# 959AI994/Multi-Gate-VAE

Hardware: NVIDIA B200
Metric: gates_per_s_fwd_bwd (higher is better)
Workload: dtype f32

## Files before the change

### multi-gate-vae_b200/csrc/mgv_tc.cuh

```cuda
#pragma once
#include <cuda_fp16.h>
#include "mgv_common.cuh"

namespace tc {

__device__ __forceinline__ uint32_t smem_u32(const void* p) { return (uint32_t)__cvta_generic_to_shared(p); }

__device__ __forceinline__ uint32_t sw128_off(int r, int c16) {
    return (uint32_t)((r >> 3) * 1024 + (r & 7) * 128 + ((c16 ^ (r & 7)) << 4));
}
__device__ __forceinline__ uint32_t plain16_off(int r, int c16) {
    return (uint32_t)((r >> 3) * 256 + c16 * 128 + (r & 7) * 16);
}

__device__ __forceinline__ uint32_t pack_f16x2_sat(float e0, float e1) {
    uint32_t r;
    asm("cvt.rn.satfinite.f16x2.f32 %0, %1, %2;" : "=r"(r) : "f"(e1), "f"(e0));
    return r;
}
__device__ __forceinline__ void split2(float a, float b, uint32_t& hi, uint32_t& lo) {
    hi = pack_f16x2_sat(a, b);
    const float2 hf = __half22float2(*reinterpret_cast<const __half2*>(&hi));
    lo = pack_f16x2_sat(a - hf.x, b - hf.y);
}
// ... 41 lines not shown
        if ((++polls & 1023u) == 0u) {
            const unsigned long long now = global_timer_ns();
            if (t0 == 0ull) t0 = now;
            else if (now - t0 > WAIT_TIMEOUT_NS) __trap();
        }
    }
};
__device__ __forceinline__ bool mbar_try_wait(uint32_t bar, uint32_t parity) {
    uint32_t done;
    asm volatile(
        "{\n\t.reg .pred p;\n\t"
        "mbarrier.try_wait.parity.shared::cta.b64 p, [%1], %2;\n\t"
        "selp.b32 %0, 1, 0, p;\n\t}"
        : "=r"(done) : "r"(bar), "r"(parity) : "memory");
    return done != 0u;
}
__device__ __forceinline__ void mbar_wait(uint32_t bar, uint32_t parity) {
    WaitGuard g;
#pragma unroll 1
    while (!mbar_try_wait(bar, parity)) g.tick();
}

__device__ __forceinline__ void mbar_wait_warp(uint32_t bar, uint32_t parity, int lane, unsigned sleep_ns = 64) {
    if (lane == 0) {
        WaitGuard g;
#pragma unroll 1
        while (!mbar_try_wait(bar, parity)) {
            if (sleep_ns) __nanosleep(sleep_ns);
            g.tick();
        }
    }
    __syncwarp();
}
__device__ __forceinline__ void mbar_wait_sleep(uint32_t bar, uint32_t parity, unsigned sleep_ns = 64) {
    WaitGuard g;
#pragma unroll 1
    while (!mbar_try_wait(bar, parity)) {
        __nanosleep(sleep_ns);
        g.tick();
    }
}

__device__ __forceinline__ void mbar_expect_tx(uint32_t bar, uint32_t bytes) {
    asm volatile("{\n\t.reg .b64 st;\n\tmbarrier.arrive.expect_tx.shared::cta.b64 st, [%0], %1;\n\t}" ::"r"(bar), "r"(bytes) : "memory");
}
__device__ __forceinline__ void bulk_g2s(uint32_t dst, const void* src, uint32_t bytes, uint32_t bar) {
    asm volatile("cp.async.bulk.shared::cluster.global.mbarrier::complete_tx::bytes [%0], [%1], %2, [%3];"
                 ::"r"(dst), "l"(src), "r"(bytes), "r"(bar) : "memory");
}

__device__ __forceinline__ void bulk_s2g(void* dst, uint32_t src, uint32_t bytes) {
    asm volatile("cp.async.bulk.global.shared::cta.bulk_group [%0], [%1], %2;" ::"l"(dst), "r"(src), "r"(bytes) : "memory");
}
__device__ __forceinline__ uint64_t l2_policy_evict_first() {
    uint64_t pol;
    asm volatile("createpolicy.fractional.L2::evict_first.b64 %0, 1.0;" : "=l"(pol));
    return pol;
}
__device__ __forceinline__ void bulk_s2g_hint(void* dst, uint32_t src, uint32_t bytes, uint64_t pol) {
    asm volatile("cp.async.bulk.global.shared::cta.bulk_group.L2::cache_hint [%0], [%1], %2, %3;" ::"l"(dst), "r"(src), "r"(bytes), "l"(pol) : "memory");
}
__device__ __forceinline__ void bulk_g2s_hint(uint32_t dst, const void* src, uint32_t bytes, uint32_t bar, uint64_t pol) {
    asm volatile("cp.async.bulk.shared::cluster.global.mbarrier::complete_tx::bytes.L2::cache_hint [%0], [%1], %2, [%3], %4;"
                 ::"r"(dst), "l"(src), "r"(bytes), "r"(bar), "l"(pol) : "memory");
}
__device__ __forceinline__ void stg_v4_hint(void* dst, const uint4& v, uint64_t pol) {
    asm volatile("st.global.L2::cache_hint.v4.b32 [%0], {%1,%2,%3,%4}, %5;" ::"l"(dst), "r"(v.x), "r"(v.y), "r"(v.z), "r"(v.w), "l"(pol) : "memory");
}
__device__ __forceinline__ void bulk_commit() { asm volatile("cp.async.bulk.commit_group;" ::: "memory"); }
__device__ __forceinline__ void bulk_wait_read0() { asm volatile("cp.async.bulk.wait_group.read 0;" ::: "memory"); }
__device__ __forceinline__ void bulk_wait0() { asm volatile("cp.async.bulk.wait_group 0;" ::: "memory"); }
__device__ __forceinline__ void named_bar_sync(int id, int nthreads) {
    asm volatile("bar.sync %0, %1;" ::"r"(id), "r"(nthreads) : "memory");
}
__device__ __forceinline__ void tmem_ld8(uint32_t taddr, float (&v)[8]) {
    uint32_t* r = reinterpret_cast<uint32_t*>(v);
    asm volatile("tcgen05.ld.sync.aligned.32x32b.x8.b32 {%0,%1,%2,%3,%4,%5,%6,%7}, [%8];"
                 : "=r"(r[0]), "=r"(r[1]), "=r"(r[2]), "=r"(r[3]), "=r"(r[4]), "=r"(r[5]), "=r"(r[6]), "=r"(r[7])
                 : "r"(taddr) : "memory");
}

__device__ __forceinline__ void fence_async_smem() { asm volatile("fence.proxy.async.shared::cta;" ::: "memory"); }
__device__ __forceinline__ void fence_before_sync() { asm volatile("tcgen05.fence::before_thread_sync;" ::: "memory"); }
__device__ __forceinline__ void fence_after_sync() { asm volatile("tcgen05.fence::after_thread_sync;" ::: "memory"); }

__device__ __forceinline__ void tmem_alloc(uint32_t* slot, uint32_t ncols) {
    asm volatile("tcgen05.alloc.cta_group::1.sync.aligned.shared::cta.b32 [%0], %1;" ::"r"(smem_u32(slot)), "r"(ncols) : "memory");
    asm volatile("tcgen05.relinquish_alloc_permit.cta_group::1.sync.aligned;" ::: "memory");
}
__device__ __forceinline__ void tmem_dealloc(uint32_t base, uint32_t ncols) {
    asm volatile("tcgen05.dealloc.cta_group::1.sync.aligned.b32 %0, %1;" ::"r"(base), "r"(ncols) : "memory");
}
__device__ __forceinline__ void tmem_ld32(uint32_t taddr, float (&v)[32]) {
    uint32_t* r = reinterpret_cast<uint32_t*>(v);
    asm volatile(
        "tcgen05.ld.sync.aligned.32x32b.x32.b32 "
        "{%0,%1,%2,%3,%4,%5,%6,%7,%8,%9,%10,%11,%12,%13,%14,%15,"
        "%16,%17,%18,%19,%20,%21,%22,%23,%24,%25,%26,%27,%28,%29,%30,%31}, [%32];"
        : "=r"(r[0]), "=r"(r[1]), "=r"(r[2]), "=r"(r[3]), "=r"(r[4]), "=r"(r[5]), "=r"(r[6]), "=r"(r[7]),
          "=r"(r[8]), "=r"(r[9]), "=r"(r[10]), "=r"(r[11]), "=r"(r[12]), "=r"(r[13]), "=r"(r[14]), "=r"(r[15]),
          "=r"(r[16]), "=r"(r[17]), "=r"(r[18]), "=r"(r[19]), "=r"(r[20]), "=r"(r[21]), "=r"(r[22]), "=r"(r[23]),
          "=r"(r[24]), "=r"(r[25]), "=r"(r[26]), "=r"(r[27]), "=r"(r[28]), "=r"(r[29]), "=r"(r[30]), "=r"(r[31])
        : "r"(taddr) : "memory");
}
__device__ __forceinline__ void tmem_ld16(uint32_t taddr, float (&v)[16]) {
    uint32_t* r = reinterpret_cast<uint32_t*>(v);
// ... 136 lines not shown
```

### multi-gate-vae_b200/csrc/struct_bwd_tc.cu

```cuda
#include <stdlib.h>
#include "struct_layout.cuh"

long long* mgv_debug_trace();
size_t mgv_struct_image_bytes(int num_enc);
int mgv_struct_build_image(const float* weights, int num_enc, uint8_t* image, int precision, cudaStream_t st);

namespace {
using namespace struct_layout;

constexpr int SGRAD = MGV_STRUCT_GRAD_FLOATS;
constexpr int EPI_WARPS = 8, GATHER_WARPS = 8;
constexpr int THREADS = (EPI_WARPS + GATHER_WARPS + 1) * 32;
constexpr int LDGS = 68;
constexpr uint32_t DG_TILE_BYTES = 131072;
constexpr int CHUNK_TILES_DEFAULT = 2048;

constexpr uint32_t S_G = A_X_LO + 4096;
constexpr uint32_t S_LN = S_G + TM * LDGS * 4;
constexpr uint32_t S_AMAX = S_LN + 512;
constexpr uint32_t S_EX = S_AMAX + 16;
constexpr uint32_t S_BAR = S_EX + 4 * 2 * TM * 4;
constexpr uint32_t S_TMEM = S_BAR + 128;
constexpr uint32_t P_SMEM = S_TMEM + 64 + 1024;
static_assert(P_SMEM <= 227 * 1024, "struct backward: shared memory");
static_assert(A_TILE_BYTES + TM * LDGS * 4 >= TM * 132 * 4, "LayerNorm gradient scratch aliases the tile + staging");
constexpr uint32_t T_ACC = 0, T_OUT = 256, T_LNP = 384;

struct BwdTC {
    int N, feat, layernorm, first, last, dir;
    int tile_beg, tile_end;
    const int* ptr;
    const int* idx;
    const int* order;
    const int* gdesc;
    const unsigned* tile_cost;
    const float* x;
    const uint8_t* image;
    const float* gout;
    const float* in_part; const float* in_agg;
    float* out_part; float* out_agg;
    const uint8_t* tiles;
    size_t tiles_enc_stride;
    uint8_t* dgbuf;
    float* scales;
    unsigned* smin;
    float* partial;
    int gxp;
    int chunk_cap;
    long long* trace;
};
#define PTRACE_MAX(slot) do { if (p.trace && it < 16) atomicMax(reinterpret_cast<unsigned long long*>(p.trace) + (((size_t)blockIdx.y * gridDim.x + blockIdx.x) * 16 + it) * 16 + (slot), (unsigned long long)clock64()); } while (0)
#define PTRACE(slot) do { if (p.trace && it < 16) p.trace[(((size_t)blockIdx.y * gridDim.x + blockIdx.x) * 16 + it) * 16 + (slot)] = clock64(); } while (0)

__device__ __forceinline__ float4 lds4(const float* p) { return *reinterpret_cast<const float4*>(p); }
__device__ __forceinline__ float pow2_scale(float amax) {
    if (!(amax > 0.f) || !isfinite(amax)) return 1.0f;
    const int e = (int)((__float_as_uint(amax) >> 23) & 0xff) - 127;
    int k = 8 - e;
    k = k < -100 ? -100 : (k > 100 ? 100 : k);
    return __uint_as_float((uint32_t)(k + 127) << 23);
}
__device__ __forceinline__ float pow2_scale_keep(float amax, float cur) {
    const float v = amax * cur;
    if (v >= 4.0f && v <= 8192.0f) return cur;
    return (amax > 0.f) ? pow2_scale(amax) : cur;
}

template <bool LOWP>
__global__ void __launch_bounds__(THREADS, 1) struct_bwd_pw_kernel(const BwdTC p) {
    extern __shared__ __align__(1024) uint8_t smem_raw[];
    const uint32_t sbase = (tc::smem_u32(smem_raw) + 1023u) & ~1023u;
    uint8_t* sgen = smem_raw + (sbase - tc::smem_u32(smem_raw));
    const int tid = threadIdx.x, lane = tid & 31, warp = tid >> 5;
    const int enc = blockIdx.y;
    const size_t eoff = (size_t)enc * p.N * D;
    const uint8_t* image = p.image + (size_t)enc * 2 * IMG_BYTES;

    const uint32_t bar_w = sbase + S_BAR, bar_a_full = bar_w + 8, bar_t_full = bar_w + 16, bar_g_empty = bar_w + 24;
    const uint32_t bar_acc_full = bar_w + 32, bar_out_full = bar_w + 40, bar_h_read = bar_w + 48, bar_dg_full = bar_w + 56;
    const uint32_t bar_dg_stored = bar_w + 64;
    uint32_t* tmem_slot = reinterpret_cast<uint32_t*>(sgen + S_TMEM);
    float* s_ln = reinterpret_cast<float*>(sgen + S_LN);
    unsigned* s_amax = reinterpret_cast<unsigned*>(sgen + S_AMAX);
    float* s_g = reinterpret_cast<float*>(sgen + S_G);

    if (tid == 0) {
        tc::mbar_init(bar_w, 1);
        tc::mbar_init(bar_a_full, GATHER_WARPS * 32);
        tc::mbar_init(bar_t_full, 1);
        tc::mbar_init(bar_g_empty, EPI_WARPS * 32);
        tc::mbar_init(bar_acc_full, 1);
        tc::mbar_init(bar_out_full, 1);
        tc::mbar_init(bar_h_read, EPI_WARPS * 32);
        tc::mbar_init(bar_dg_full, EPI_WARPS * 32);
        tc::mbar_init(bar_dg_stored, EPI_WARPS * 32);
        tc::fence_barrier_init();
        tc::mbar_expect_tx(bar_w, IMG_W);
#pragma unroll 1
        for (uint32_t o = 0; o < IMG_W; o += 16384u) tc::bulk_g2s(sbase + o, image + o, 16384u, bar_w);
    }
    if (tid < 2 * D) s_ln[tid] = __ldg(reinterpret_cast<const float*>(image + IMG_W) + tid);
    if (tid < 4) s_amax[tid] = 0u;
    if (warp == 0) tc::tmem_alloc(tmem_slot, 512);
    const int tile_beg = p.tile_beg + (int)blockIdx.x, tile_end = p.tile_end, tile_step = (int)gridDim.x;
    tc::fence_before_sync();
    __syncthreads();
    tc::fence_after_sync();
    const uint32_t tmem = *tmem_slot;

    if (warp >= EPI_WARPS && warp < EPI_WARPS + GATHER_WARPS) {
        const int gw = warp - EPI_WARPS, rg = lane >> 3, c = lane & 7;
        const int4* gdesc = reinterpret_cast<const int4*>(p.gdesc);
        const float* gsrc = p.last ? p.gout + eoff : p.in_part + eoff;
        const float* asrc = p.in_agg + eoff;
        const bool nbg = !p.last;
        int4 dn[4];
#pragma unroll
        for (int ps = 0; ps < 4; ++ps) {
            const int r = tile_beg * TM + gw * 16 + ps * 4 + rg;
            dn[ps] = (tile_beg < tile_end && r < p.N) ? __ldg(gdesc + r) : make_int4(-1, 0, 0, 0);
        }
        int it = 0;
        for (int tile = tile_beg; tile < tile_end; tile += tile_step, ++it) {
            if (lane == 0) PTRACE_MAX(13);
            int4 dc[4];
#pragma unroll
            for (int ps = 0; ps < 4; ++ps) dc[ps] = dn[ps];
#pragma unroll
            for (int ps = 0; ps < 4; ++ps) {
                const int r = (tile + tile_step) * TM + gw * 16 + ps * 4 + rg;
                dn[ps] = (tile + tile_step < tile_end && r < p.N) ? __ldg(gdesc + r) : make_int4(-1, 0, 0, 0);
            }
#pragma unroll
            for (int hf = 0; hf < 2; ++hf) {
                int node[2], beg[2], cnt[2], jn[2];
                float4 g[2][2], va[2][2];
                int maxc = 0;
                const float4 z4 = make_float4(0.f, 0.f, 0.f, 0.f);
#pragma unroll
                for (int q = 0; q < 2; ++q) {
                    const int4 d = dc[2 * hf + q];
                    node[q] = d.x; beg[q] = d.y; cnt[q] = nbg ? d.z : 0; jn[q] = d.w;
                    maxc = max(maxc, cnt[q]);
                    g[q][0] = z4; g[q][1] = z4; va[q][0] = z4; va[q][1] = z4;
                    if (node[q] >= 0) {
                        g[q][0] = mgv_ld4(gsrc + (size_t)node[q] * D + c * 8);
                        g[q][1] = mgv_ld4(gsrc + (size_t)node[q] * D + c * 8 + 4);
                    }
                    if (cnt[q] > 0) {
                        va[q][0] = mgv_ld4(asrc + (size_t)jn[q] * D + c * 8);
                        va[q][1] = mgv_ld4(asrc + (size_t)jn[q] * D + c * 8 + 4);
                    }
                    if (cnt[q] > 1) jn[q] = p.idx[beg[q] + 1] & NODE_MASK;
                }
                float ag[2][8];
#pragma unroll
                for (int q = 0; q < 2; ++q) {
                    ag[q][0] = g[q][0].x + va[q][0].x; ag[q][1] = g[q][0].y + va[q][0].y; ag[q][2] = g[q][0].z + va[q][0].z; ag[q][3] = g[q][0].w + va[q][0].w;
                    ag[q][4] = g[q][1].x + va[q][1].x; ag[q][5] = g[q][1].y + va[q][1].y; ag[q][6] = g[q][1].z + va[q][1].z; ag[q][7] = g[q][1].w + va[q][1].w;
                }
                for (int sl = 1; sl < maxc; sl += 2) {
                    int j[2][2];
#pragma unroll
                    for (int q = 0; q < 2; ++q) {
                        j[q][0] = jn[q];
                        j[q][1] = (sl + 1 < cnt[q]) ? (p.idx[beg[q] + sl + 1] & NODE_MASK) : 0;
                        if (sl + 2 < cnt[q]) jn[q] = p.idx[beg[q] + sl + 2] & NODE_MASK;
                    }
                    float4 wa[2][2][2];
#pragma unroll
                    for (int q = 0; q < 2; ++q)
#pragma unroll
                        for (int t = 0; t < 2; ++t) {
                            wa[q][t][0] = z4; wa[q][t][1] = z4;
                            if (sl + t < cnt[q]) {
                                wa[q][t][0] = mgv_ld4(asrc + (size_t)j[q][t] * D + c * 8);
                                wa[q][t][1] = mgv_ld4(asrc + (size_t)j[q][t] * D + c * 8 + 4);
                            }
                        }
#pragma unroll
                    for (int q = 0; q < 2; ++q)
#pragma unroll
                        for (int t = 0; t < 2; ++t) {
                            ag[q][0] += wa[q][t][0].x; ag[q][1] += wa[q][t][0].y; ag[q][2] += wa[q][t][0].z; ag[q][3] += wa[q][t][0].w;
                            ag[q][4] += wa[q][t][1].x; ag[q][5] += wa[q][t][1].y; ag[q][6] += wa[q][t][1].z; ag[q][7] += wa[q][t][1].w;
                        }
                }
                if (hf == 0) {
                    if (lane == 0) PTRACE_MAX(14);
                    tc::mbar_wait_warp(bar_g_empty, (uint32_t)((it & 1) ^ 1), lane, 64);
                }
#pragma unroll
                for (int q = 0; q < 2; ++q) {
                    float* dst = s_g + (gw * 16 + (2 * hf + q) * 4 + rg) * LDGS + c * 8;
                    *reinterpret_cast<float4*>(dst) = make_float4(ag[q][0], ag[q][1], ag[q][2], ag[q][3]);
                    *reinterpret_cast<float4*>(dst + 4) = make_float4(ag[q][4], ag[q][5], ag[q][6], ag[q][7]);
                }
            }
            tc::mbar_arrive(bar_a_full);
            if (lane == 0) PTRACE_MAX(15);
        }
    } else if (warp == EPI_WARPS + GATHER_WARPS) {
        if (lane == 0 && tile_beg < tile_end) {
            auto load_tile = [&](int t) {
                const uint8_t* src = p.tiles + (size_t)enc * p.tiles_enc_stride + (size_t)t * A_TILE_BYTES;
                if (LOWP) {
                    tc::mbar_expect_tx(bar_t_full, 36864u);
#pragma unroll 1
                    for (uint32_t o = 0; o < 16384u; o += 8192u) {
                        tc::bulk_g2s(sbase + A_AGG_HI + o, src + o, 8192u, bar_t_full);
                        tc::bulk_g2s(sbase + A_H_HI + o, src + (A_H_HI - A_AGG_HI) + o, 8192u, bar_t_full);
                    }
                    tc::bulk_g2s(sbase + A_X_HI, src + (A_X_HI - A_AGG_HI), 4096u, bar_t_full);
                } else {
                    tc::mbar_expect_tx(bar_t_full, A_TILE_BYTES);
#pragma unroll 1
                    for (uint32_t o = 0; o < A_TILE_BYTES; o += 8192u) tc::bulk_g2s(sbase + A_AGG_HI + o, src + o, 8192u, bar_t_full);
                }
            };
            auto issue_recompute = [&](uint32_t tph) {
                tc::mbar_wait_sleep(bar_t_full, tph, 32);
                tc::fence_after_sync();
                const uint32_t d = tmem + T_ACC;
                tc::mma3p<LOWP>(d, tc::desc_k_plain16(sbase + A_X_HI), tc::desc_k_plain16(sbase + A_X_LO),
                         tc::desc_k_plain16(sbase + WX_HI), tc::desc_k_plain16(sbase + WX_LO), tc::make_idesc(128, 256, false, false, LOWP), 0u);
#pragma unroll
                for (int j = 0; j < 4; ++j)
                    tc::mma3p<LOWP>(d, tc::desc_k_sw128(sbase + A_H_HI + 32 * j), tc::desc_k_sw128(sbase + A_H_LO + 32 * j),
                             tc::desc_k_sw128(sbase + WHH_HI + 32 * j), tc::desc_k_sw128(sbase + WHH_LO + 32 * j),
                             tc::make_idesc(128, 128, false, false, LOWP), 1u);
#pragma unroll
                for (int j = 0; j < 4; ++j)
                    tc::mma3p<LOWP>(d + 192u, tc::desc_k_sw128(sbase + A_H_HI + 32 * j), tc::desc_k_sw128(sbase + A_H_LO + 32 * j),
                             tc::desc_k_sw128(sbase + WHH_HI + 16384 + 32 * j), tc::desc_k_sw128(sbase + WHH_LO + 16384 + 32 * j),
                             tc::make_idesc(128, 64, false, false, LOWP), 1u);
#pragma unroll
                for (int j = 0; j < 4; ++j)
                    tc::mma3p<LOWP>(d, tc::desc_k_sw128(sbase + A_AGG_HI + 32 * j), tc::desc_k_sw128(sbase + A_AGG_LO + 32 * j),
                             tc::desc_k_sw128(sbase + WC_HI + 32 * j), tc::desc_k_sw128(sbase + WC_LO + 32 * j),
                             tc::make_idesc(128, 192, false, false, LOWP), 1u);
                tc::mma_commit(bar_acc_full);
            };
            tc::mbar_wait_sleep(bar_w, 0u);
            load_tile(tile_beg);
            issue_recompute(0u);
            int it = 0;
            for (int tile = tile_beg; tile < tile_end; tile += tile_step, ++it) {
                const uint32_t ph = (uint32_t)(it & 1);
                tc::mbar_wait_sleep(bar_acc_full, ph, 32);
                tc::mbar_wait_sleep(bar_h_read, ph, 32);
                if (tile + tile_step < tile_end) load_tile(tile + tile_step);
                tc::mbar_wait_sleep(bar_dg_full, ph, 32);
                tc::fence_after_sync();
                PTRACE(7);
                if (!p.first) {
                    const uint32_t o = tmem + T_OUT;
                    const uint32_t i128 = tc::make_idesc(128, 128, false, true, LOWP), i64 = tc::make_idesc(128, 64, false, true, LOWP);
#pragma unroll
                    for (int s = 0; s < 8; ++s) {
                        const uint32_t a = tmem + T_ACC + 16u * s;
                        tc::mma3p_ts<LOWP>(o, a, a + 8u, tc::desc_mn_sw128(sbase + WC_HI + 2048u * s, WHH_HI - WC_HI),
                                            tc::desc_mn_sw128(sbase + WC_LO + 2048u * s, WHH_LO - WC_LO), i128, 1u);
                    }
#pragma unroll
                    for (int s = 8; s < 12; ++s) {
                        const uint32_t a = tmem + T_ACC + 16u * s;
                        tc::mma3p_ts<LOWP>(o, a, a + 8u, tc::desc_mn_sw128(sbase + WC_HI + 2048u * s, 0),
                                            tc::desc_mn_sw128(sbase + WC_LO + 2048u * s, 0), i64, 1u);
                    }
#pragma unroll
                    for (int s = 12; s < 16; ++s) {
                        const uint32_t a = tmem + T_ACC + 16u * s;
                        tc::mma3p_ts<LOWP>(o + 64u, a, a + 8u, tc::desc_mn_sw128(sbase + WHH_HI + 2048u * (s - 4), 0),
                                            tc::desc_mn_sw128(sbase + WHH_LO + 2048u * (s - 4), 0), i64, 1u);
                    }
                    tc::mma_commit(bar_out_full);
                }
                if (tile + tile_step < tile_end) {
                    tc::mbar_wait_sleep(bar_dg_stored, ph, 32);
                    issue_recompute(ph ^ 1u);
                }
                PTRACE(3);
            }
        }
    } else if (warp < EPI_WARPS) {
        const int wg = warp >> 2, row = (warp & 3) * 32 + lane, u0 = 32 * wg;
        const uint32_t tl = tmem + ((uint32_t)((warp & 3) * 32) << 16);
        const uint32_t t_acc = tl + T_ACC, t_out = tl + T_OUT, t_lnp = tl + T_LNP;
        const float* gs = s_g + row * LDGS;
        float* s_ex = reinterpret_cast<float*>(sgen + S_EX);
        constexpr int EPI_T = EPI_WARPS * 32;
#pragma unroll 1
        for (int cc = 0; cc < 32; cc += 4) {
            tc::tmem_st4(t_lnp + u0 + cc, 0.f, 0.f, 0.f, 0.f);
            tc::tmem_st4(t_lnp + 64 + u0 + cc, 0.f, 0.f, 0.f, 0.f);
        }
        tc::tmem_st_wait();
        float run_scale = 1.0f;
        const uint64_t pol_stream = tc::l2_policy_evict_first();
        int it = 0;
        for (int tile = tile_beg; tile < tile_end; tile += tile_step, ++it) {
            const uint32_t ph = (uint32_t)(it & 1);
            const bool valid = tile * TM + row < p.N;
            const int node = valid ? p.order[tile * TM + row] : 0;
            tc::mbar_wait_warp(bar_t_full, ph, lane, 32);
#pragma unroll
            for (int c8 = 0; c8 < 4; ++c8) {
                const uint32_t off = tc::sw128_off(row, 4 * wg + c8);
                const uint4 hi = *reinterpret_cast<const uint4*>(sgen + A_H_HI + off);
                float h[8];
                if (LOWP) {
                    const uint32_t* w = reinterpret_cast<const uint32_t*>(&hi);
#pragma unroll
                    for (int e = 0; e < 4; ++e) { h[2 * e] = __uint_as_float(w[e] << 16); h[2 * e + 1] = __uint_as_float(w[e] & 0xffff0000u); }
                } else {
                    const uint4 lo = *reinterpret_cast<const uint4*>(sgen + A_H_LO + off);
                    const __half2* h2 = reinterpret_cast<const __half2*>(&hi);
                    const __half2* l2 = reinterpret_cast<const __half2*>(&lo);
#pragma unroll
                    for (int e = 0; e < 4; ++e) {
                        const float2 a = __half22float2(h2[e]), bq = __half22float2(l2[e]);
                        h[2 * e] = a.x + bq.x; h[2 * e + 1] = a.y + bq.y;
                    }
                }
                tc::tmem_st8f(t_out + u0 + 8 * c8, h);
            }
            tc::mbar_arrive(bar_h_read);
            tc::mbar_wait_warp(bar_acc_full, ph, lane, 32);
            tc::mbar_wait_warp(bar_a_full, ph, lane, 32);
            tc::fence_after_sync();
            tc::tmem_st_wait();
            if (tid == 0) PTRACE(4);
            float sum = 0.f;
#pragma unroll 1
            for (int c8 = 0; c8 < 4; ++c8) {
                const int u = u0 + 8 * c8;
                float gr[8], gz[8], gi[8], gh[8], h[8];
                tc::tmem_ld8(t_acc + u, gr);
                tc::tmem_ld8(t_acc + 64 + u, gz);
                tc::tmem_ld8(t_acc + 128 + u, gi);
                tc::tmem_ld8(t_acc + 192 + u, gh);
                tc::tmem_ld8(t_out + u, h);
                tc::tmem_ld_wait();
#pragma unroll
                for (int e = 0; e < 8; ++e) {
                    float r, z, n, hn;
                    gru_gates(gr[e], gz[e], gi[e], gh[e], r, z, n, hn);
                    gr[e] = r; gz[e] = z; gi[e] = n;
                    h[e] = fmaf(z, h[e] - n, n);
                    sum += h[e];
                }
                tc::tmem_st8f(t_acc + u, gr);
                tc::tmem_st8f(t_acc + 64 + u, gz);
                tc::tmem_st8f(t_acc + 128 + u, gi);
// ... 151 lines not shown
                    tc::stg_v4_hint(hb + 3072, make_uint4(qk[4], qk[5], qk[6], qk[7]), pol_stream);
                    if (!LOWP) {
                        tc::stg_v4_hint(hb + 65536, make_uint4(pk[8], pk[9], pk[10], pk[11]), pol_stream);
                        tc::stg_v4_hint(hb + 65536 + 1024, make_uint4(pk[12], pk[13], pk[14], pk[15]), pol_stream);
                        tc::stg_v4_hint(hb + 65536 + 2048, make_uint4(qk[8], qk[9], qk[10], qk[11]), pol_stream);
                        tc::stg_v4_hint(hb + 65536 + 3072, make_uint4(qk[12], qk[13], qk[14], qk[15]), pol_stream);
                    }
                }
            }
            tc::fence_before_sync();
            tc::mbar_arrive(bar_dg_stored);
            if (!p.first) {
                tc::mbar_wait_warp(bar_out_full, ph, lane, 32);
                tc::fence_after_sync();
                if (tid == 0) PTRACE(8);
                const float inv = 1.0f / scale;
#pragma unroll 2
                for (int c8 = 0; c8 < 4; ++c8) {
                    const int u = u0 + 8 * c8;
                    float a[8], q[8];
                    tc::tmem_ld8(t_out + u, a);
                    tc::tmem_ld8(t_out + 64 + u, q);
                    tc::tmem_ld_wait();
#pragma unroll
                    for (int e = 0; e < 8; ++e) { a[e] *= inv; q[e] *= inv; }
                    if (valid) {
                        stg8(p.out_agg + eoff + (size_t)node * D + u, a);
                        stg8(p.out_part + eoff + (size_t)node * D + u, q);
                    }
                }
            }
            if (tid == 0) PTRACE(9);
        }
    }
    tc::fence_before_sync();
    __syncthreads();
    tc::fence_after_sync();
    float* scratch = reinterpret_cast<float*>(sgen + A_AGG_HI);
    if (warp < EPI_WARPS) {
        const int row = (warp & 3) * 32 + lane, u0 = 32 * (warp >> 2);
        const uint32_t t_lnp = tmem + ((uint32_t)((warp & 3) * 32) << 16) + T_LNP;
#pragma unroll 1
        for (int c8 = 0; c8 < 8; ++c8) {
            const int col = (c8 < 4) ? u0 + 8 * c8 : 64 + u0 + 8 * (c8 - 4);
            float v[8];
            tc::tmem_ld8(t_lnp + col, v);
            tc::tmem_ld_wait();
            *reinterpret_cast<float4*>(scratch + row * 132 + col) = make_float4(v[0], v[1], v[2], v[3]);
            *reinterpret_cast<float4*>(scratch + row * 132 + col + 4) = make_float4(v[4], v[5], v[6], v[7]);
        }
    }
    tc::fence_before_sync();
    __syncthreads();
    if (tid < 2 * D && p.layernorm && tile_beg < tile_end) {
        float s = 0.f;
#pragma unroll 8
        for (int r = 0; r < TM; ++r) s += scratch[r * 132 + tid];
        float* part = p.partial + (((size_t)enc * p.gxp + blockIdx.x) * 2 + p.dir) * SGRAD;
        part[O_LNW + tid] += s;
    }
    if (warp == 0) tc::tmem_dealloc(tmem, 512);
}

__device__ __forceinline__ void red_add4(float4* dst, const float4& v) {
    asm volatile("red.global.add.v4.f32 [%0], {%1,%2,%3,%4};" ::"l"(dst), "f"(v.x), "f"(v.y), "f"(v.z), "f"(v.w) : "memory");
}

constexpr int W_THREADS = 6 * 32;
constexpr uint32_t ST_DG_HI = 0, ST_DG_LO = 32768, ST_AGG_HI = 65536, ST_H_HI = 73728, ST_AGG_LO = 81920, ST_H_LO = 90112;
constexpr uint32_t ST_X_HI = 98304, ST_X_LO = 100352, ST_BYTES = 102400;
constexpr uint32_t W_BAR = 2 * ST_BYTES;
constexpr uint32_t W_TMEM = W_BAR + 64;
constexpr uint32_t W_SMEM = W_TMEM + 64 + 1024;
static_assert(W_SMEM <= 227 * 1024, "struct weight gradient: shared memory");

struct WgTC {
    int ntiles;
    int chunk_cap;
    int dir, gxp;
    const uint8_t* tiles;
    size_t tiles_enc_stride;
    int tile_base;
    const uint8_t* dgbuf;
    const float* scales;
    const unsigned* smin;
    float* partial;
    long long* trace;
};
#define WTRACE(slot) do { if (p.trace && i < 16) p.trace[(((size_t)blockIdx.y * gridDim.x + blockIdx.x) * 16 + i) * 16 + (slot)] = clock64(); } while (0)

template <bool LOWP>
__global__ void __launch_bounds__(W_THREADS, 1) struct_bwd_wgrad_kernel(const WgTC p) {
    extern __shared__ __align__(1024) uint8_t smem_raw[];
    const uint32_t sbase = (tc::smem_u32(smem_raw) + 1023u) & ~1023u;
    uint8_t* sgen = smem_raw + (sbase - tc::smem_u32(smem_raw));
    const int tid = threadIdx.x, lane = tid & 31, warp = tid >> 5;
    const int enc = blockIdx.y;
    const uint32_t bar_full = sbase + W_BAR, bar_ready = bar_full + 16, bar_empty = bar_full + 32, bar_done = bar_full + 48;
    uint32_t* tmem_slot = reinterpret_cast<uint32_t*>(sgen + W_TMEM);
    if (tid == 0) {
        for (int s = 0; s < 2; ++s) {
            tc::mbar_init(bar_full + 8 * s, 1);
            tc::mbar_init(bar_ready + 8 * s, 4 * 32);
            tc::mbar_init(bar_empty + 8 * s, 1);
        }
        tc::mbar_init(bar_done, 1);
        tc::fence_barrier_init();
    }
    if (warp == 0) tc::tmem_alloc(tmem_slot, 512);
    tc::fence_before_sync();
    __syncthreads();
    tc::fence_after_sync();
    const uint32_t tmem = *tmem_slot;
    const int tile_beg = (int)((long long)p.ntiles * blockIdx.x / gridDim.x);
    const int tile_end = (int)((long long)p.ntiles * (blockIdx.x + 1) / gridDim.x);
    const int nhalf = 2 * (tile_end - tile_beg);
    const float smin = __uint_as_float(p.smin[enc]);

    if (warp == 0) {
        if (lane == 0) {
            const uint64_t pol = tc::l2_policy_evict_first();
            for (int i = 0; i < nhalf; ++i) {
                const int s = i & 1, tile = tile_beg + (i >> 1), h = i & 1;
                WTRACE(0);
                tc::mbar_wait_sleep(bar_empty + 8 * s, (uint32_t)(((i >> 1) & 1) ^ 1));
                WTRACE(1);
                tc::mbar_expect_tx(bar_full + 8 * s, LOWP ? 51200u : ST_BYTES);
                const uint8_t* dg = p.dgbuf + ((size_t)enc * p.chunk_cap + tile) * DG_TILE_BYTES + (size_t)h * 32768;
                const uint8_t* at = p.tiles + (size_t)enc * p.tiles_enc_stride + (size_t)(p.tile_base + tile) * A_TILE_BYTES;
                const uint32_t st = sbase + (uint32_t)s * ST_BYTES, bar = bar_full + 8 * s;
                tc::bulk_g2s_hint(st + ST_DG_HI, dg, 16384u, bar, pol);
                tc::bulk_g2s_hint(st + ST_DG_HI + 16384u, dg + 16384, 16384u, bar, pol);
                tc::bulk_g2s_hint(st + ST_AGG_HI, at + 0 + h * 8192, 8192u, bar, pol);
                tc::bulk_g2s_hint(st + ST_H_HI, at + 32768 + h * 8192, 8192u, bar, pol);
                tc::bulk_g2s_hint(st + ST_X_HI, at + 65536 + h * 2048, 2048u, bar, pol);
                if (!LOWP) {
                    tc::bulk_g2s_hint(st + ST_DG_LO, dg + 65536, 16384u, bar, pol);
                    tc::bulk_g2s_hint(st + ST_DG_LO + 16384u, dg + 65536 + 16384, 16384u, bar, pol);
                    tc::bulk_g2s_hint(st + ST_AGG_LO, at + 16384 + h * 8192, 8192u, bar, pol);
                    tc::bulk_g2s_hint(st + ST_H_LO, at + 49152 + h * 8192, 8192u, bar, pol);
                    tc::bulk_g2s_hint(st + ST_X_LO, at + 69632 + h * 2048, 2048u, bar, pol);
                }
            }
        }
    } else if (warp == 1) {
        if (lane == 0) {
            const uint32_t i128 = tc::make_idesc(128, 128, true, true, LOWP), i16 = tc::make_idesc(128, 16, true, true, LOWP);
            for (int i = 0; i < nhalf; ++i) {
                const int s = i & 1;
                WTRACE(4);
                tc::mbar_wait_sleep(bar_ready + 8 * s, (uint32_t)((i >> 1) & 1), 32);
                tc::fence_after_sync();
                WTRACE(5);
                const uint32_t st = sbase + (uint32_t)s * ST_BYTES;
#pragma unroll
                for (int j = 0; j < 4; ++j) {
                    const uint32_t acc = (i > 0 || j > 0) ? 1u : 0u;
                    const uint64_t b_hi = tc::desc_mn_sw128(st + ST_AGG_HI + 2048u * j, 8192), b_lo = tc::desc_mn_sw128(st + ST_AGG_LO + 2048u * j, 8192);
                    const uint64_t x_hi = tc::desc_mn_plain16(st + ST_X_HI + 512u * j), x_lo = tc::desc_mn_plain16(st + ST_X_LO + 512u * j);
#pragma unroll
                    for (int g = 0; g < 2; ++g) {
                        const uint64_t a_hi = tc::make_desc(st + ST_DG_HI + 16384u * g + 256u * j, 128, 1024, tc::LAYOUT_NONE);
                        const uint64_t a_lo = tc::make_desc(st + ST_DG_LO + 16384u * g + 256u * j, 128, 1024, tc::LAYOUT_NONE);
                        tc::mma3p<LOWP>(tmem + 160u * g, a_hi, a_lo, b_hi, b_lo, i128, acc);
                        tc::mma3p<LOWP>(tmem + 160u * g + 128u, a_hi, a_lo, x_hi, x_lo, i16, acc);
                    }
// ... 53 lines not shown
            for (int q = t128; q < G3 * 19; q += 128) {
                const int o = q / 19, c4 = q % 19;
                if (c4 < 18) {
                    const int g = o >= 128 ? 1 : 0, col = c4 < 16 ? 4 * c4 : 128 + 4 * (c4 - 16);
                    const float4 v = *reinterpret_cast<const float4*>(stg + (g * 128 + o - 128 * g) * FLD + col);
                    red_add4(part4 + (O_WCX + o * LDC) / 4 + c4, v);
                }
            }
            for (int q = t128; q < G3 * 17; q += 128) {
                const int o = q / 17, c4 = q % 17;
                if (c4 < 16) {
                    const int row = o >= 128 ? 128 + o - 64 : o;
                    const float4 v = *reinterpret_cast<const float4*>(stg + row * FLD + 64 + 4 * c4);
                    red_add4(part4 + (O_WHH + o * LDM) / 4 + c4, v);
                }
            }
            for (int o = t128; o < G3; o += 128) {
                const int rc = o >= 128 ? 128 + o - 128 : o, rh = o >= 128 ? 128 + o - 64 : o;
                atomicAdd(part + O_BC + o, stg[rc * FLD + 136]);
                atomicAdd(part + O_BIH + o, stg[rc * FLD + 137]);
                atomicAdd(part + O_BHH + o, stg[rh * FLD + 137]);
            }
            if (tid == 64) WTRACE(10);
        }
    }
    tc::fence_before_sync();
    __syncthreads();
    if (warp == 0) tc::tmem_dealloc(tmem, 512);
}

__global__ void struct_reduce_tc_kernel(const float* __restrict__ partial, int gxp, float* __restrict__ grads, int num_enc) {
    const size_t total = (size_t)num_enc * 2 * SGRAD;
    const size_t idx = (size_t)blockIdx.x * blockDim.x + threadIdx.x;
    if (idx >= total) return;
    const int enc = (int)(idx / (2 * SGRAD));
    const size_t rem = idx % (2 * (size_t)SGRAD);
    float s = 0.f;
    for (int b = 0; b < gxp; ++b) s += partial[((size_t)enc * gxp + b) * 2 * SGRAD + rem];
    grads[idx] = s;
}

__global__ void fill_u32_kernel(unsigned* p, unsigned v, int n) {
    const int i = blockIdx.x * blockDim.x + threadIdx.x;
    if (i < n) p[i] = v;
}

int sm_count(int* sms) {
    int dev = 0;
    MGV_CUDA(cudaGetDevice(&dev));
    MGV_CUDA(cudaDeviceGetAttribute(sms, cudaDevAttrMultiProcessorCount, dev));
    return MGV_OK;
}

int chunk_tiles() {
    const char* e = getenv("MGV_STRUCT_CHUNK");
    const int v = e ? atoi(e) : 0;
    return v > 0 ? v : CHUNK_TILES_DEFAULT;
}

}

extern "C" size_t mgv_struct_bwd_workspace_bytes(int64_t N, int32_t num_enc) {
    int sms = 148;
    sm_count(&sms);
    const int64_t ntiles = (N + TM - 1) / TM;
    const int CHUNK_TILES = chunk_tiles();
    const int64_t cap = ntiles < CHUNK_TILES ? ntiles : CHUNK_TILES;
    size_t b = mgv_struct_image_bytes(num_enc) + 256;
    b += 4 * mgv_align_up((size_t)num_enc * N * D * 4 + 256, 256);
    b += mgv_align_up((size_t)sms * 2 * SGRAD * 4 + 256, 256);
    b += mgv_align_up((size_t)num_enc * cap * DG_TILE_BYTES + 1024, 1024);
    b += mgv_align_up((size_t)num_enc * cap * 4 + 256, 256);
    const int64_t chunks = (ntiles + CHUNK_TILES - 1) / CHUNK_TILES;
    b += mgv_align_up((size_t)(chunks > 0 ? chunks : 1) * 2 * 4 + 256, 256) + 4096;
    return b;
}

extern "C" int mgv_struct_encoder_bwd(const mgv_schedule* sch, int32_t num_enc, int32_t rounds, int32_t layernorm,
                                      int32_t feat, const float* x, const float* weights, const void* tiles,
                                      const float* gout, float* grads, void* ws, size_t ws_bytes,
                                      int32_t precision, mgv_stream_t stream) {
    cudaStream_t st = (cudaStream_t)stream;
    MGV_REQUIRE(sch != nullptr, "struct encoder: null schedule");
    MGV_REQUIRE(num_enc >= 1 && num_enc <= 2, "struct encoder: num_enc must be 1 or 2");
    MGV_REQUIRE(rounds >= 1, "struct encoder: rounds must be >= 1");
    MGV_REQUIRE(feat >= 0 && feat <= MGV_MAX_FEAT, "struct encoder: dim_feature %d > %d", feat, MGV_MAX_FEAT);
    const int N = sch->N;
    MGV_CUDA(cudaMemsetAsync(grads, 0, (size_t)num_enc * 2 * SGRAD * sizeof(float), st));
    if (N == 0) return MGV_OK;
    MGV_REQUIRE(sch->deg_order_in && sch->deg_order_out && sch->tile_cost_in && sch->tile_cost_out && sch->gdesc_in && sch->gdesc_out,
                "struct encoder: the schedule carries no degree order (mgv_build_degree_order)");
    MGV_REQUIRE(tiles != nullptr, "mgv_struct_encoder_bwd: the operand tiles saved by mgv_struct_encoder_fwd are required (tiles == NULL)");
    if (ws_bytes < mgv_struct_bwd_workspace_bytes(N, num_enc)) {
        mgv_set_error("mgv_struct_encoder_bwd: workspace %zu < %zu bytes", ws_bytes, mgv_struct_bwd_workspace_bytes(N, num_enc));
        return MGV_ERR_WORKSPACE;
    }
    int sms = 0;
    int rc = sm_count(&sms);
    if (rc != MGV_OK) return rc;
    const int ntiles = (N + TM - 1) / TM;
    const int CHUNK_TILES = chunk_tiles();
    const int cap = ntiles < CHUNK_TILES ? ntiles : CHUNK_TILES;
    const int chunks = (ntiles + CHUNK_TILES - 1) / CHUNK_TILES;
    const int gxp = sms / num_enc > 0 ? sms / num_enc : 1;
    const int steps = 2 * rounds;
    const size_t slot = (size_t)N * D;

    MgvArena a(ws, ws_bytes);
    uint8_t* image = a.take<uint8_t>((size_t)num_enc * 2 * IMG_BYTES);
    float* part[2];
    float* agg[2];
    part[0] = a.take<float>((size_t)num_enc * slot); part[1] = a.take<float>((size_t)num_enc * slot);
    agg[0] = a.take<float>((size_t)num_enc * slot); agg[1] = a.take<float>((size_t)num_enc * slot);
    float* partial = a.take<float>((size_t)num_enc * gxp * 2 * SGRAD);
    a.off = mgv_align_up(a.off, 1024);
    uint8_t* dgbuf = a.take<uint8_t>((size_t)num_enc * cap * DG_TILE_BYTES);
    float* scales = a.take<float>((size_t)num_enc * cap);
    unsigned* smin = a.take<unsigned>((size_t)chunks * 2);
    MGV_REQUIRE(a.ok(), "mgv_struct_encoder_bwd: workspace layout overflow");
    MGV_REQUIRE(precision == 0 || precision == 1, "struct encoder: precision must be 0 (fp32-accurate) or 1 (bf16)");
    rc = mgv_struct_build_image(weights, num_enc, image, precision, st);
    if (rc != MGV_OK) return rc;
    MGV_CUDA(cudaMemsetAsync(partial, 0, (size_t)num_enc * gxp * 2 * SGRAD * sizeof(float), st));
    const bool lowp = precision == 1;
    const void* pw_fn = lowp ? (const void*)struct_bwd_pw_kernel<true> : (const void*)struct_bwd_pw_kernel<false>;
    const void* wg_fn = lowp ? (const void*)struct_bwd_wgrad_kernel<true> : (const void*)struct_bwd_wgrad_kernel<false>;
    MGV_CUDA(cudaFuncSetAttribute(pw_fn, cudaFuncAttributeMaxDynamicSharedMemorySize, (int)P_SMEM));
    MGV_CUDA(cudaFuncSetAttribute(wg_fn, cudaFuncAttributeMaxDynamicSharedMemorySize, (int)W_SMEM));

    for (int k = steps; k >= 1; --k) {
        const int dir = (k & 1) ? 0 : 1;
        fill_u32_kernel<<<(chunks * 2 + 63) / 64, 64, 0, st>>>(smin, 0x7f000000u, chunks * 2);
        mgv_count_launches(1);
        for (int ch = 0; ch < chunks; ++ch) {
            const int tb = ch * CHUNK_TILES, te = (tb + CHUNK_TILES < ntiles) ? tb + CHUNK_TILES : ntiles;
            int gx = gxp;
            if (gx > te - tb) gx = te - tb;
            BwdTC p{};
            p.N = N; p.feat = feat; p.layernorm = layernorm; p.first = (k == 1); p.last = (k == steps); p.dir = dir;
            p.tile_beg = tb; p.tile_end = te;
            p.ptr = dir == 0 ? sch->in_ptr : sch->out_ptr;
            p.idx = dir == 0 ? sch->in_src : sch->out_pack;
            p.order = dir == 0 ? sch->deg_order_in : sch->deg_order_out;
            p.gdesc = dir == 0 ? sch->gdesc_in : sch->gdesc_out;
            p.tile_cost = dir == 0 ? sch->tile_cost_in : sch->tile_cost_out;
            p.x = x;
            p.image = image + (size_t)dir * IMG_BYTES;
            p.gout = gout;
            p.in_part = part[k & 1]; p.in_agg = agg[k & 1];
            p.out_part = part[(k - 1) & 1]; p.out_agg = agg[(k - 1) & 1];
            p.tiles = (const uint8_t*)tiles + (size_t)(k - 1) * ntiles * A_TILE_BYTES;
            p.tiles_enc_stride = (size_t)steps * ntiles * A_TILE_BYTES;
            p.dgbuf = dgbuf; p.scales = scales; p.smin = smin + 2 * ch;
            p.partial = partial; p.gxp = gxp; p.chunk_cap = cap;
            p.trace = (k == 2 && ch == 0 && !getenv("MGV_TRACE_WGRAD")) ? mgv_debug_trace() : nullptr;
            if (lowp) struct_bwd_pw_kernel<true><<<dim3(gx, num_enc), THREADS, P_SMEM, st>>>(p);
            else struct_bwd_pw_kernel<false><<<dim3(gx, num_enc), THREADS, P_SMEM, st>>>(p);
            WgTC w{};
            w.ntiles = te - tb; w.chunk_cap = cap; w.dir = dir; w.gxp = gxp;
            w.tiles = p.tiles; w.tiles_enc_stride = p.tiles_enc_stride; w.tile_base = tb;
            w.dgbuf = dgbuf; w.scales = scales; w.smin = smin + 2 * ch; w.partial = partial;
            w.trace = (k == 2 && ch == 0 && getenv("MGV_TRACE_WGRAD")) ? mgv_debug_trace() : nullptr;
            if (lowp) struct_bwd_wgrad_kernel<true><<<dim3(gx, num_enc), W_THREADS, W_SMEM, st>>>(w);
            else struct_bwd_wgrad_kernel<false><<<dim3(gx, num_enc), W_THREADS, W_SMEM, st>>>(w);
            mgv_count_launches(2);
        }
    }
    const size_t total = (size_t)num_enc * 2 * SGRAD;
    struct_reduce_tc_kernel<<<(unsigned)((total + 255) / 256), 256, 0, st>>>(partial, gxp, grads, num_enc);
    mgv_count_launches(1);
    return mgv_check_cuda(cudaGetLastError(), "mgv_struct_encoder_bwd");
}
```

Measured before the change: 19.01 million.

## Use programmatic dependent launch and remove per-step smin fill kernel

Launches the backward pointwise and wgrad kernels with programmatic stream serialization, so each kernel's prologue (barrier init, weight image bulk load, TMEM alloc) overlaps the tail of the previous kernel before griddepcontrol.wait. The per-step fill kernel is replaced by double-buffered smin slots, with the next step's slot reset inside the pointwise kernel. Tile assignment also changes so the remainder tiles go to the last blocks in reversed order, which may balance the last wave differently. The risk is ordering: the reset of smin_next and the early launch_dependents must not race with readers of the previous slot.

Measured after the change: 19.62 million, median of 6. 1.03x the previous value.

```diff
diff --git a/multi-gate-vae_b200/csrc/mgv_tc.cuh b/multi-gate-vae_b200/csrc/mgv_tc.cuh
--- a/multi-gate-vae_b200/csrc/mgv_tc.cuh
+++ b/multi-gate-vae_b200/csrc/mgv_tc.cuh
@@ -117,6 +117,8 @@
 __device__ __forceinline__ void bulk_s2g(void* dst, uint32_t src, uint32_t bytes) {
     asm volatile("cp.async.bulk.global.shared::cta.bulk_group [%0], [%1], %2;" ::"l"(dst), "r"(src), "r"(bytes) : "memory");
 }
+__device__ __forceinline__ void grid_dep_wait() { asm volatile("griddepcontrol.wait;" ::: "memory"); }
+__device__ __forceinline__ void grid_dep_launch() { asm volatile("griddepcontrol.launch_dependents;" ::: "memory"); }
 __device__ __forceinline__ uint64_t l2_policy_evict_first() {
     uint64_t pol;
     asm volatile("createpolicy.fractional.L2::evict_first.b64 %0, 1.0;" : "=l"(pol));
diff --git a/multi-gate-vae_b200/csrc/struct_bwd_tc.cu b/multi-gate-vae_b200/csrc/struct_bwd_tc.cu
--- a/multi-gate-vae_b200/csrc/struct_bwd_tc.cu
+++ b/multi-gate-vae_b200/csrc/struct_bwd_tc.cu
@@ -44,6 +44,7 @@
     uint8_t* dgbuf;
     float* scales;
     unsigned* smin;
+    unsigned* smin_next;
     float* partial;
     int gxp;
     int chunk_cap;
@@ -102,11 +103,16 @@
     if (tid < 2 * D) s_ln[tid] = __ldg(reinterpret_cast<const float*>(image + IMG_W) + tid);
     if (tid < 4) s_amax[tid] = 0u;
     if (warp == 0) tc::tmem_alloc(tmem_slot, 512);
-    const int tile_beg = p.tile_beg + (int)blockIdx.x, tile_end = p.tile_end, tile_step = (int)gridDim.x;
+    const int gx = (int)gridDim.x, bx = (int)blockIdx.x, nt = p.tile_end - p.tile_beg, full = nt / gx, rem = nt % gx;
+    const int ntl = full + (bx >= gx - rem ? 1 : 0);
+    auto tile_of = [&](int i) { return p.tile_beg + (i < full ? bx + i * gx : full * gx + (gx - 1 - bx)); };
     tc::fence_before_sync();
     __syncthreads();
     tc::fence_after_sync();
     const uint32_t tmem = *tmem_slot;
+    tc::grid_dep_wait();
+    tc::grid_dep_launch();
+    if (tid == 0 && blockIdx.x == 0) p.smin_next[enc] = 0x7f000000u;
 
     if (warp >= EPI_WARPS && warp < EPI_WARPS + GATHER_WARPS) {
         const int gw = warp - EPI_WARPS, rg = lane >> 3, c = lane & 7;
@@ -117,19 +123,19 @@
         int4 dn[4];
 #pragma unroll
         for (int ps = 0; ps < 4; ++ps) {
-            const int r = tile_beg * TM + gw * 16 + ps * 4 + rg;
-            dn[ps] = (tile_beg < tile_end && r < p.N) ? __ldg(gdesc + r) : make_int4(-1, 0, 0, 0);
+            const int r = tile_of(0) * TM + gw * 16 + ps * 4 + rg;
+            dn[ps] = (ntl > 0 && r < p.N) ? __ldg(gdesc + r) : make_int4(-1, 0, 0, 0);
         }
         int it = 0;
-        for (int tile = tile_beg; tile < tile_end; tile += tile_step, ++it) {
+        for (; it < ntl; ++it) {
             if (lane == 0) PTRACE_MAX(13);
             int4 dc[4];
 #pragma unroll
             for (int ps = 0; ps < 4; ++ps) dc[ps] = dn[ps];
 #pragma unroll
             for (int ps = 0; ps < 4; ++ps) {
-                const int r = (tile + tile_step) * TM + gw * 16 + ps * 4 + rg;
-                dn[ps] = (tile + tile_step < tile_end && r < p.N) ? __ldg(gdesc + r) : make_int4(-1, 0, 0, 0);
+                const int r = tile_of(it + 1) * TM + gw * 16 + ps * 4 + rg;
+                dn[ps] = (it + 1 < ntl && r < p.N) ? __ldg(gdesc + r) : make_int4(-1, 0, 0, 0);
             }
 #pragma unroll
             for (int hf = 0; hf < 2; ++hf) {
@@ -201,7 +207,7 @@
             if (lane == 0) PTRACE_MAX(15);
         }
     } else if (warp == EPI_WARPS + GATHER_WARPS) {
-        if (lane == 0 && tile_beg < tile_end) {
+        if (lane == 0 && ntl > 0) {
             auto load_tile = [&](int t) {
                 const uint8_t* src = p.tiles + (size_t)enc * p.tiles_enc_stride + (size_t)t * A_TILE_BYTES;
                 if (LOWP) {
@@ -242,14 +248,14 @@
                 tc::mma_commit(bar_acc_full);
             };
             tc::mbar_wait_sleep(bar_w, 0u);
-            load_tile(tile_beg);
+            load_tile(tile_of(0));
             issue_recompute(0u);
             int it = 0;
-            for (int tile = tile_beg; tile < tile_end; tile += tile_step, ++it) {
+            for (; it < ntl; ++it) {
                 const uint32_t ph = (uint32_t)(it & 1);
                 tc::mbar_wait_sleep(bar_acc_full, ph, 32);
                 tc::mbar_wait_sleep(bar_h_read, ph, 32);
-                if (tile + tile_step < tile_end) load_tile(tile + tile_step);
+                if (it + 1 < ntl) load_tile(tile_of(it + 1));
                 tc::mbar_wait_sleep(bar_dg_full, ph, 32);
                 tc::fence_after_sync();
                 PTRACE(7);
@@ -276,7 +282,7 @@
                     }
                     tc::mma_commit(bar_out_full);
                 }
-                if (tile + tile_step < tile_end) {
+                if (it + 1 < ntl) {
                     tc::mbar_wait_sleep(bar_dg_stored, ph, 32);
                     issue_recompute(ph ^ 1u);
                 }
@@ -299,7 +305,8 @@
         float run_scale = 1.0f;
         const uint64_t pol_stream = tc::l2_policy_evict_first();
         int it = 0;
-        for (int tile = tile_beg; tile < tile_end; tile += tile_step, ++it) {
+        for (; it < ntl; ++it) {
+            const int tile = tile_of(it);
             const uint32_t ph = (uint32_t)(it & 1);
             const bool valid = tile * TM + row < p.N;
             const int node = valid ? p.order[tile * TM + row] : 0;
@@ -557,7 +564,7 @@
     }
     tc::fence_before_sync();
     __syncthreads();
-    if (tid < 2 * D && p.layernorm && tile_beg < tile_end) {
+    if (tid < 2 * D && p.layernorm && ntl > 0) {
         float s = 0.f;
 #pragma unroll 8
         for (int r = 0; r < TM; ++r) s += scratch[r * 132 + tid];
@@ -617,6 +624,8 @@
     __syncthreads();
     tc::fence_after_sync();
     const uint32_t tmem = *tmem_slot;
+    tc::grid_dep_wait();
+    tc::grid_dep_launch();
     const int tile_beg = (int)((long long)p.ntiles * blockIdx.x / gridDim.x);
     const int tile_end = (int)((long long)p.ntiles * (blockIdx.x + 1) / gridDim.x);
     const int nhalf = 2 * (tile_end - tile_beg);
@@ -776,6 +785,21 @@
     return MGV_OK;
 }
 
+template <typename P>
+cudaError_t launch(void (*kern)(P), dim3 grid, int threads, size_t smem, cudaStream_t st, bool pdl, const P& p) {
+    cudaLaunchConfig_t cfg = {};
+    cfg.gridDim = grid;
+    cfg.blockDim = dim3(threads);
+    cfg.dynamicSmemBytes = smem;
+    cfg.stream = st;
+    cudaLaunchAttribute at[1];
+    at[0].id = cudaLaunchAttributeProgrammaticStreamSerialization;
+    at[0].val.programmaticStreamSerializationAllowed = 1;
+    cfg.attrs = at;
+    cfg.numAttrs = pdl ? 1 : 0;
+    return cudaLaunchKernelEx(&cfg, kern, p);
+}
+
 int chunk_tiles() {
     const char* e = getenv("MGV_STRUCT_CHUNK");
     const int v = e ? atoi(e) : 0;
@@ -796,7 +820,7 @@
     b += mgv_align_up((size_t)num_enc * cap * DG_TILE_BYTES + 1024, 1024);
     b += mgv_align_up((size_t)num_enc * cap * 4 + 256, 256);
     const int64_t chunks = (ntiles + CHUNK_TILES - 1) / CHUNK_TILES;
-    b += mgv_align_up((size_t)(chunks > 0 ? chunks : 1) * 2 * 4 + 256, 256) + 4096;
+    b += mgv_align_up((size_t)(chunks > 0 ? chunks : 1) * 2 * 2 * 4 + 256, 256) + 4096;
     return b;
 }
 
@@ -840,7 +864,7 @@
     a.off = mgv_align_up(a.off, 1024);
     uint8_t* dgbuf = a.take<uint8_t>((size_t)num_enc * cap * DG_TILE_BYTES);
     float* scales = a.take<float>((size_t)num_enc * cap);
-    unsigned* smin = a.take<unsigned>((size_t)chunks * 2);
+    unsigned* smin = a.take<unsigned>((size_t)2 * chunks * 2);
     MGV_REQUIRE(a.ok(), "mgv_struct_encoder_bwd: workspace layout overflow");
     MGV_REQUIRE(precision == 0 || precision == 1, "struct encoder: precision must be 0 (fp32-accurate) or 1 (bf16)");
     rc = mgv_struct_build_image(weights, num_enc, image, precision, st);
@@ -852,10 +876,10 @@
     MGV_CUDA(cudaFuncSetAttribute(pw_fn, cudaFuncAttributeMaxDynamicSharedMemorySize, (int)P_SMEM));
     MGV_CUDA(cudaFuncSetAttribute(wg_fn, cudaFuncAttributeMaxDynamicSharedMemorySize, (int)W_SMEM));
 
+    fill_u32_kernel<<<(2 * chunks * 2 + 63) / 64, 64, 0, st>>>(smin, 0x7f000000u, 2 * chunks * 2);
+    mgv_count_launches(1);
     for (int k = steps; k >= 1; --k) {
         const int dir = (k & 1) ? 0 : 1;
-        fill_u32_kernel<<<(chunks * 2 + 63) / 64, 64, 0, st>>>(smin, 0x7f000000u, chunks * 2);
-        mgv_count_launches(1);
         for (int ch = 0; ch < chunks; ++ch) {
             const int tb = ch * CHUNK_TILES, te = (tb + CHUNK_TILES < ntiles) ? tb + CHUNK_TILES : ntiles;
             int gx = gxp;
@@ -875,18 +899,18 @@
             p.out_part = part[(k - 1) & 1]; p.out_agg = agg[(k - 1) & 1];
             p.tiles = (const uint8_t*)tiles + (size_t)(k - 1) * ntiles * A_TILE_BYTES;
             p.tiles_enc_stride = (size_t)steps * ntiles * A_TILE_BYTES;
-            p.dgbuf = dgbuf; p.scales = scales; p.smin = smin + 2 * ch;
+            p.dgbuf = dgbuf; p.scales = scales; p.smin = smin + (size_t)(k & 1) * chunks * 2 + 2 * ch;
+            p.smin_next = smin + (size_t)((k - 1) & 1) * chunks * 2 + 2 * ch;
             p.partial = partial; p.gxp = gxp; p.chunk_cap = cap;
             p.trace = (k == 2 && ch == 0 && !getenv("MGV_TRACE_WGRAD")) ? mgv_debug_trace() : nullptr;
-            if (lowp) struct_bwd_pw_kernel<true><<<dim3(gx, num_enc), THREADS, P_SMEM, st>>>(p);
-            else struct_bwd_pw_kernel<false><<<dim3(gx, num_enc), THREADS, P_SMEM, st>>>(p);
+            const bool pdl = !(k == steps && ch == 0);
+            MGV_CUDA(launch(lowp ? struct_bwd_pw_kernel<true> : struct_bwd_pw_kernel<false>, dim3(gx, num_enc), THREADS, P_SMEM, st, pdl, p));
             WgTC w{};
             w.ntiles = te - tb; w.chunk_cap = cap; w.dir = dir; w.gxp = gxp;
             w.tiles = p.tiles; w.tiles_enc_stride = p.tiles_enc_stride; w.tile_base = tb;
-            w.dgbuf = dgbuf; w.scales = scales; w.smin = smin + 2 * ch; w.partial = partial;
+            w.dgbuf = dgbuf; w.scales = scales; w.smin = p.smin; w.partial = partial;
             w.trace = (k == 2 && ch == 0 && getenv("MGV_TRACE_WGRAD")) ? mgv_debug_trace() : nullptr;
-            if (lowp) struct_bwd_wgrad_kernel<true><<<dim3(gx, num_enc), W_THREADS, W_SMEM, st>>>(w);
-            else struct_bwd_wgrad_kernel<false><<<dim3(gx, num_enc), W_THREADS, W_SMEM, st>>>(w);
+            MGV_CUDA(launch(lowp ? struct_bwd_wgrad_kernel<true> : struct_bwd_wgrad_kernel<false>, dim3(gx, num_enc), W_THREADS, W_SMEM, st, true, w));
             mgv_count_launches(2);
         }
     }
```
